# KatiaJDL/CenterPoly

Hardware: AMD Instinct MI355X
Metric: inference img/s @2048x1024 DLA-34 (1 GPU) (higher is better)
Workload: dtype f32 I/O; split-bf16 x3 contraction (a*b ~ ah*bh + ah*bl + al*bh on bf16 MFMA, ~2^-16 per product) in the convolutions, the heads and DCNv2; f32 accumulate; 1 GPU; BASELINE config 2: DLA-34 + DCNv2, 1x3x1024x2048 synthetic, 16-vertex cartesian head, K=128, forward + sigmoid + NMS/top-k/decode; parallelism=single

## Files before the change

### centerpoly_amd/_C.py

```python
import ctypes
import os
from ctypes import POINTER, Structure, c_char_p, c_float, c_int32, c_int64, c_size_t, c_void_p

import torch

_HERE = os.path.dirname(os.path.abspath(__file__))
LIB_PATH = os.path.join(_HERE, "csrc", "libcenterpoly_hip.so")

CP_OK = 0
REP = {"cartesian": 0, "polar": 1, "polar_fixed": 2}
HEATMAP_UMICH, HEATMAP_ELLIPSE = 0, 1
L1_PLAIN, L1_POLAR, L1_POLAR_FIXED, L1_RELU20, L1_SMOOTH = 0, 1, 2, 3, 4
DCN_BWD_EXACT_F32, DCN_BWD_NARROW_TILES = 1, 2
DCN_CONTRACTION = {"f32": 0, "bf16x3": 1, "bf16x3_region": 3}


class DcnShape(Structure):
    _fields_ = [(n, c_int32) for n in ("B", "Cin", "H", "W", "Cout", "kh", "kw", "stride", "pad",
                                       "dil", "deformable_groups")]


class TargetShape(Structure):
    _fields_ = [(n, c_int32) for n in ("B", "max_objs", "nbr_points", "num_classes", "out_h", "out_w",
                                       "rep", "no_reorder_flip")]
# ... 76 lines not shown
    "cp_polydet_targets_ex": (c_int32, [POINTER(TargetShape), c_int32] + [_P] * 19 + [_P, c_size_t, _P]),
    "cp_polydet_dense_targets": (c_int32, [POINTER(TargetShape), _P, _P, c_size_t, _P, _P, _P]),
    "cp_conv_direct_supported": (c_int32, [c_int32] * 5),
    "cp_conv_direct_wgrad_supported": (c_int32, [c_int32] * 5),
    "cp_conv_direct_wgrad": (c_int32, [_P, _P, _P] + [c_int32] * 8 + [_P]),
    "cp_conv_direct_forward": (c_int32, [_P, _P, _P, _P] + [c_int32] * 9 + [_P]),
    "cp_conv_direct_forward_ex": (c_int32, [_P, _P, _P, _P] + [c_int32] * 10 + [_P]),
    "cp_conv3x3_mfma_supported": (c_int32, [c_int32] * 4),
    "cp_conv3x3_mfma_weight_bytes": (c_size_t, [c_int32] * 2),
    "cp_conv3x3_mfma_prepare": (c_int32, [_P, c_int32, c_int32, c_int32, _P, _P]),
    "cp_conv3x3_mfma_forward": (c_int32, [_P, _P, _P, _P, _P] + [c_int32] * 6 + [_P]),
    "cp_conv_mfma_weight_bytes": (c_size_t, [c_int32] * 3),
    "cp_conv_mfma_prepare": (c_int32, [_P, c_int32, c_int32, c_int32, c_int32, _P, _P]),
    "cp_conv3x3_s2_wgrad_supported": (c_int32, [c_int32] * 4),
    "cp_conv3x3_s2_wgrad": (c_int32, [_P, _P, _P] + [c_int32] * 5 + [_P]),
    "cp_conv7x7_c3_supported": (c_int32, [c_int32] * 4),
    "cp_conv7x7_c3_weight_bytes": (c_size_t, [c_int32]),
    "cp_conv7x7_c3_prepare": (c_int32, [_P, c_int32, _P, _P]),
    "cp_conv7x7_c3_forward": (c_int32, [_P, _P, _P, _P] + [c_int32] * 6 + [_P]),
    "cp_conv_mfma_prepare_blocks": (c_int32, [c_int32] * 3),
    "cp_conv_mfma_prepare_batch": (c_int32, [_P, c_int32, c_int32, _P]),
    "cp_conv_mfma_forward": (c_int32, [_P, _P, c_int32, _P, _P, _P, _P] + [c_int32] * 6 + [_P]),
    "cp_conv_mfma_forward_strided": (c_int32, [_P, _P, c_int32, _P, _P, _P, _P] + [c_int32] * 7 + [_P]),
    "cp_dla_base_pair_supported": (c_int32, [c_int32] * 2),
    "cp_dla_base_pair_forward": (c_int32, [_P] * 6 + [c_int32] * 3 + [_P]),
    "cp_conv_mfma_forward_split": (c_int32, [_P, c_int32, _P, _P, _P, _P] + [c_int32] * 9 + [_P]),
    "cp_activation_split": (c_int32, [_P, _P] + [c_int32] * 4 + [_P]),
    "cp_activation_unsplit": (c_int32, [_P, _P] + [c_int32] * 4 + [_P]),
    "cp_conv_mfma_input_grad_relu_workspace_bytes": (c_size_t, [c_int32] * 4),
    "cp_conv_mfma_input_grad_relu": (c_int32, [_P] * 5 + [c_int32] * 6 + [_P, c_size_t, _P]),
    "cp_conv3x3_s2_input_grad": (c_int32, [_P, _P, _P, _P] + [c_int32] * 5 + [_P]),
    "cp_conv3x3_mfma_wgrad_supported": (c_int32, [c_int32] * 4),
    "cp_conv3x3_mfma_wgrad": (c_int32, [_P, _P, _P] + [c_int32] * 5 + [_P]),
    "cp_conv_mfma_wgrad": (c_int32, [_P, _P, _P] + [c_int32] * 6 + [_P]),
    "cp_heads_fused_w2_bytes": (c_size_t, [c_int32]),
    "cp_heads_fused_prepare_w2": (c_int32, [_P, c_int32, c_int32, _P, _P]),
    "cp_heads_fused_forward": (c_int32, [_P, _P, _P, _P, _P, _P, _P] + [c_int32] * 6 + [_P]),
    "cp_maxpool2x2_forward": (c_int32, [_P, _P] + [c_int32] * 4 + [_P]),
    "cp_maxpool2x2_backward": (c_int32, [_P, _P, _P] + [c_int32] * 4 + [_P]),
    "cp_conv1x1_act_forward": (c_int32, [_P, c_int64, _P, c_int32, _P, _P, _P, c_int32, c_int32, c_int32, c_int64, _P]),
    "cp_soft_nms": (c_int32, [_P, c_int32, c_int32, c_float, c_float, c_float, c_int32]),
    "cp_soft_nms_device": (c_int32, [_P, c_int32, _P, _P, c_int32, c_float, c_float, c_float, c_int32, _P, _P]),
    "cp_merge_detections_workspace_bytes": (c_size_t, [c_int32] * 4),
    "cp_merge_detections": (c_int32, [_P] + [c_int32] * 6 + [c_float] * 3 + [c_int32, _P, _P, _P, c_size_t, _P]),
    "cp_polydet_decode_workspace_bytes": (c_size_t, [c_int32] * 5),
    "cp_polydet_decode": (c_int32, [_P, _P, _P, _P] + [c_int32] * 7 + [_P, _P, _P, _P, c_size_t, _P]),
# ... 138 lines not shown
```

### centerpoly_amd/csrc/conv_mfma.hip

```cpp
#include "cp_common.h"

#include <type_traits>

namespace {

typedef __bf16 bf16x8 __attribute__((ext_vector_type(8)));
typedef __bf16 bf16x4 __attribute__((ext_vector_type(4)));
typedef unsigned u32x4 __attribute__((ext_vector_type(4)));
typedef unsigned u32x2 __attribute__((ext_vector_type(2)));

#ifndef CP_CVABL
#define CP_CVABL 0
#endif
#ifdef CP_CVSTAMP
#define CVSTAMP(i) do { if ((i) < 16) stamp[i] = __builtin_amdgcn_s_memtime(); } while (0)
#else
#define CVSTAMP(i) do { } while (0)
#endif
constexpr int KC = 32;
constexpr int TW = 32;
constexpr unsigned OOB = 0xFFFFFFF0u;

__device__ __forceinline__ void wperm_element(const float* __restrict__ w, bf16x8* __restrict__ wp, int M, int K, int nchunk,
                                              int taps, int transposed, int e) {
  const int lane = e & 63;
  int r = e >> 6;
  const int hl = r & 1;
  r >>= 1;
  const int tap = r % taps;
  r /= taps;
  const int chunk = r % nchunk, ct = r / nchunk;
  const int m = ct * 16 + (lane & 15);
  bf16x8 o;
#pragma unroll
  for (int j = 0; j < 8; ++j) {
    const int k = chunk * KC + 8 * (lane >> 4) + j;
    float v = 0.f;
    if (m < M && k < K) {
      if (transposed == 6) {
        v = w[((long long)k * M + m) * 9 + tap];
// ... 33 lines not shown
  v += dpp(v, std::integral_constant<int, 0xB1>{});
  v += dpp(v, std::integral_constant<int, 0x4E>{});
  v += dpp(v, std::integral_constant<int, 0x141>{});
  v += dpp(v, std::integral_constant<int, 0x140>{});
  return v;
}

constexpr int MAXSRC = 4;
struct CvArgs {
  const float* xsrc[MAXSRC];
  int csrc[MAXSRC];
  const bf16x8* wp;
  const float* bias;
  const float* res;
  float* out;
  int Cin, H, W, Ho, Wo, Cout, nchunk, ncot, tiles_x, relu;
  const float* mask;
  float* colsum;
  int Hf, Wf;
  const bf16x8* xpre = nullptr;
  long long pre_plane = 0;
  int out_split = 0;
  long long out_plane = 0;
};

template <int MT, int RW, int TAPS, int KS = 1, int ST = 1, bool IG2 = false, bool PRE = false, bool OSPLIT = false>
__global__ __launch_bounds__(256 * KS, KS > 1 ? (ST > 1 && TAPS == 9 ? 1 : 4) : 2) void conv_mfma_kernel(CvArgs a) {
  static_assert(!IG2 || (TAPS == 9 && KS == 1 && ST == 1), "IG2: 3x3, stride-1 staging, no split-K");
  static_assert(!PRE || (TAPS == 9 && ST == 1 && !IG2), "PRE: 3x3 / stride 1 forward");
  static_assert(!OSPLIT || !IG2, "split planes out: forward forms");
  constexpr bool TRD = !IG2 && !OSPLIT;
  constexpr int NCLS = IG2 ? 4 : 1;
#ifdef CP_CVSTAMP
  unsigned long long stamp[16];
  const unsigned long long rt0 = __builtin_amdgcn_s_memrealtime();
  int sti = 1;
#endif
  CVSTAMP(0);
  constexpr int S = TAPS == 1 ? 1 : ST;
  constexpr int SUB = TAPS == 1 ? ST : 1;
  constexpr int HALO = TAPS == 9 ? 1 : 0, LW = S * TW + (TAPS == 9 ? 3 : 1) - S;
  constexpr int TH = 4 * RW, LH = S * TH + (TAPS == 9 ? 3 : 1) - S, NT = 2 * RW, PLANE = 4 * LH * LW;
  constexpr int UNITS = PLANE, ITERS = (UNITS + 255) / 256, SB = ITERS <= 6 ? ITERS : 5;
  constexpr int RED = (KS - 1) * 256 * MT * NT;
  constexpr int XS_F = KS * 2 * PLANE;
  __shared__ bf16x8 Xall[XS_F > RED ? XS_F : RED];
// ... 30 lines not shown
  f32x4 (&acc)[MT][NT] = accs[0];

  const long long tstride = (long long)a.nchunk * TAPS * 2 * 64;
  const bf16x8* wq = a.wp + (long long)cot * MT * tstride + lane;
  bf16x8 af[MT][2];
  {
    const bf16x8* fq = wq + (long long)(min(grp, a.nchunk - 1) * TAPS * 2) * 64;
#pragma unroll
    for (int m = 0; m < MT; ++m) {
      af[m][0] = fq[m * tstride];
      af[m][1] = fq[m * tstride + 64];
    }
  }

  const int bbase = (g * LH + S * wid * RW) * LW + S * c;

  int src = 0, src_c0 = 0;
  auto load = [&](int chunk, int i0, auto& v) {
    while (src + 1 < MAXSRC && chunk * KC >= src_c0 + a.csrc[src] && a.csrc[src + 1] > 0) {
      src_c0 += a.csrc[src];
      ++src;
    }
    const int cs = a.csrc[src];
    const __amdgpu_buffer_rsrc_t rs_x = __builtin_amdgcn_make_buffer_rsrc(
        const_cast<float*>(a.xsrc[src] + (long long)b * cs * HW), 0, (int)((unsigned)cs * (unsigned)HW * 4u), 0x00020000);
    const unsigned cb = (unsigned)(chunk * KC - src_c0) * cstep;
    constexpr int N = sizeof(v) / sizeof(v[0]);
#pragma unroll
    for (int i = 0; i < N; ++i) {
      const unsigned o = (i0 + i >= ITERS || soff[(i0 + i) % ITERS] == OOB) ? OOB : soff[(i0 + i) % ITERS] + cb;
#pragma unroll
      for (int j = 0; j < 8; ++j)
        v[i][j] = (CP_CVABL & 2) ? (float)(o + j) : __builtin_bit_cast(
            float, __builtin_amdgcn_raw_buffer_load_b32(rs_x, o == OOB ? OOB : o + j * cstep, 0, 0));
    }
  };
  auto store = [&](int i0, auto& v) {
    constexpr int N = sizeof(v) / sizeof(v[0]);
#pragma unroll
    for (int i = 0; i < N; ++i) {
      const int u = tid + (i0 + i) * 256;
      if (i0 + i < ITERS && u < UNITS) {
        bf16x8 h, l;
#pragma unroll
        for (int j = 0; j < 8; ++j) {
          const __bf16 hh = (__bf16)v[i][j];
          h[j] = hh;
          l[j] = (__bf16)(v[i][j] - (float)hh);
        }
        Xs[u] = h;
// ... 18 lines not shown
    }
  };
  auto store_pre = [&](int i0, auto& vh, auto& vl) {
    constexpr int N = sizeof(vh) / sizeof(vh[0]);
#pragma unroll
    for (int i = 0; i < N; ++i) {
      const int u = tid + (i0 + i) * 256;
      if (i0 + i < ITERS && u < UNITS) {
        Xs[u] = __builtin_bit_cast(bf16x8, vh[i]);
        Xs[PLANE + u] = __builtin_bit_cast(bf16x8, vl[i]);
      }
    }
  };
  auto bread = [&](int tap, bf16x8 (&bh)[NT], bf16x8 (&bl)[NT]) {
    const int dy = IG2 ? (tap / 3 == 0 ? 2 : 1) : tap / 3, dx = IG2 ? (tap % 3 == 0 ? 2 : 1) : tap % 3;
#pragma unroll
    for (int n = 0; n < NT; ++n) {
      const int idx = bbase + (S * (n >> 1) + dy) * LW + S * (n & 1) * 16 + dx;
      bh[n] = (CP_CVABL & 4) ? af[n % MT][0] : Xs[idx];
      bl[n] = (CP_CVABL & 4) ? af[n % MT][1] : Xs[PLANE + idx];
    }
  };

  for (int chunk = grp; chunk - grp < a.nchunk; chunk += KS) {
    const bool active = chunk < a.nchunk;
    __syncthreads();
#ifdef CP_CVSTAMP
    CVSTAMP(sti); ++sti;
#endif
    if (active && !(CP_CVABL & 16)) {
#pragma unroll
      for (int i0 = 0; i0 < ITERS; i0 += SB) {
        if constexpr (PRE) {
          u32x4 vh[SB], vl[SB];
          load_pre(chunk, i0, vh, vl);
          store_pre(i0, vh, vl);
        } else {
          float v[SB][8];
          load(chunk, i0, v);
          store(i0, v);
        }
      }
    }
#ifdef CP_CVSTAMP
    CVSTAMP(sti); ++sti;
#endif
    __syncthreads();
#ifdef CP_CVSTAMP
    CVSTAMP(sti); ++sti;
#endif
    if (!active) continue;

#pragma unroll
    for (int tap = 0; tap < TAPS; ++tap) {
      const int cls = IG2 ? (tap / 3 != 1) * 2 + (tap % 3 != 1) : 0;
      bf16x8 an[MT][2];
      {
        const int nfrag = tap < TAPS - 1 ? chunk * TAPS + tap + 1
                                         : (chunk + KS < a.nchunk ? (chunk + KS) * TAPS : chunk * TAPS + tap);
        const bf16x8* nq = wq + (long long)(nfrag * 2) * 64;
#pragma unroll
        for (int m = 0; m < MT; ++m) {
          an[m][0] = (CP_CVABL & 1) ? af[m][0] : nq[m * tstride];
          an[m][1] = (CP_CVABL & 1) ? af[m][1] : nq[m * tstride + 64];
        }
      }
      {
        bf16x8 bh[NT], bl[NT];
        bread(tap, bh, bl);
#pragma unroll
        for (int m = 0; m < MT; ++m)
#pragma unroll
          for (int n = 0; n < NT; ++n) {
            f32x4& d = accs[cls][m][n];
// ... 284 lines not shown
      else if (Cout <= 32 && wgs(2, 16) >= 448) launch(conv_mfma_kernel<2, 4, 9, 1, 1, false, PRE, OS>, 2, 16, 1);
      else if (wgs(2, 8) >= 320) launch(conv_mfma_kernel<2, 2, 9, 1, 1, false, PRE, OS>, 2, 8, 1);
      else if (wgs(2, 4) < 384 && a.nchunk >= 8) launch(conv_mfma_kernel<2, 1, 9, 4, 1, false, PRE, OS>, 2, 4, 4);
      else if (wgs(2, 4) < 768 && a.nchunk >= 4) launch(conv_mfma_kernel<2, 1, 9, 2, 1, false, PRE, OS>, 2, 4, 2);
      else launch(conv_mfma_kernel<2, 1, 9, 1, 1, false, PRE, OS>, 2, 4, 1);
    };
    if (a.xpre && a.out_split) pick(std::true_type{}, std::true_type{});
    else if (a.xpre) pick(std::true_type{}, std::false_type{});
    else if (a.out_split) pick(std::false_type{}, std::true_type{});
    else pick(std::false_type{}, std::false_type{});
  } else {
    if (Cout > 32 && wgs(4, 8) >= 448) launch(conv_mfma_kernel<4, 2, 1>, 4, 8, 1);
    else if (wgs(2, 8) >= 320) launch(conv_mfma_kernel<2, 2, 1>, 2, 8, 1);
    else if (wgs(2, 4) < 384 && a.nchunk >= 8) launch(conv_mfma_kernel<2, 1, 1, 4>, 2, 4, 4);
    else if (wgs(2, 4) < 768 && a.nchunk >= 4) launch(conv_mfma_kernel<2, 1, 1, 2>, 2, 4, 2);
    else launch(conv_mfma_kernel<2, 1, 1>, 2, 4, 1);
  }
  return cp_launch_status();
}

static int conv_forward_impl(const float* const* xs, const int32_t* cs, int32_t nsrc, const void* wperm, const float* bias,
                             const float* residual, const float* mask, float* colsum, float* out, int32_t B, int32_t H,
                             int32_t W, int32_t Cout, int32_t taps, int32_t stride, int32_t relu, void* stream,
                             int* tiles_out = nullptr, int x_split = 0, int out_split = 0) {
  hipStream_t st = (hipStream_t)stream;
  CP_CHECK_ARG(xs && cs && wperm && out && B >= 1 && nsrc >= 1 && nsrc <= MAXSRC && (taps == 1 || taps == 9));
  if (stride != 1 && stride != 2) return CP_EUNSUPPORTED;
  CvArgs a;
  int Cin = 0;
  for (int i = 0; i < MAXSRC; ++i) {
    a.xsrc[i] = i < nsrc ? xs[i] : nullptr;
    a.csrc[i] = i < nsrc ? cs[i] : 0;
    if (i < nsrc) {
      CP_CHECK_ARG(xs[i] && cs[i] >= 1);
      if (nsrc > 1 && cs[i] % KC != 0) return CP_EUNSUPPORTED;
      if (!cp_conv3x3_mfma_supported(cs[i], Cout, H, W)) return CP_EUNSUPPORTED;
      Cin += cs[i];
    }
  }
  a.wp = (const bf16x8*)wperm;
  a.bias = bias;
  a.res = residual;
  a.out = out;
  a.Cin = Cin;
  a.H = H;
  a.W = W;
  a.Cout = Cout;
  a.Ho = (H - 1) / stride + 1;
  a.Wo = (W - 1) / stride + 1;
  a.nchunk = (Cin + KC - 1) / KC;
  a.tiles_x = (a.Wo + TW - 1) / TW;
  a.relu = relu;
  a.Hf = a.Ho; a.Wf = a.Wo;
  a.mask = mask; a.colsum = colsum;
  if ((long long)a.Ho * a.Wo * 64 * 4 >= 0x7FFFFFF0ll) return CP_EUNSUPPORTED;
  if (x_split) {
    if (nsrc != 1 || taps != 9 || stride != 1 || Cin % KC != 0) return CP_EUNSUPPORTED;
    a.xpre = reinterpret_cast<const bf16x8*>(xs[0]);
    a.pre_plane = (long long)B * (Cin / 8) * H * W;
// ... 47 lines not shown
  CP_CHECK_ARG(x && in && B >= 1 && C >= 8 && H >= 1 && W >= 1);
  if (C % 8 != 0) return CP_EUNSUPPORTED;
  const long long HW = (long long)H * W, plane = (long long)B * (C / 8) * HW;
  if (plane >= 0x7FFFFFFFll * 256) return CP_EUNSUPPORTED;
  hipLaunchKernelGGL(activation_unsplit_kernel, dim3((unsigned)((plane + 255) / 256)), dim3(256), 0, (hipStream_t)stream,
                     (const bf16x8*)in, x, HW, plane);
  return cp_launch_status();
}

int cp_conv_mfma_forward_split(const void* x, int32_t x_split, const void* wperm, const float* bias, const float* residual,
                               void* out, int32_t out_split, int32_t B, int32_t Cin, int32_t H, int32_t W, int32_t Cout,
                               int32_t taps, int32_t stride, int32_t relu, void* stream) {
  const float* xs[1] = {reinterpret_cast<const float*>(x)};
  const int32_t cs[1] = {Cin};
  return conv_forward_impl(xs, cs, 1, wperm, bias, residual, nullptr, nullptr, reinterpret_cast<float*>(out), B, H, W, Cout,
                           taps, stride, relu, stream, nullptr, x_split ? 1 : 0, out_split ? 1 : 0);
}

int cp_conv_mfma_forward_strided(const float* const* xs, const int32_t* cs, int32_t nsrc, const void* wperm,
                                 const float* bias, const float* residual, float* out, int32_t B, int32_t H, int32_t W,
                                 int32_t Cout, int32_t taps, int32_t stride, int32_t relu, void* stream) {
  return conv_forward_impl(xs, cs, nsrc, wperm, bias, residual, nullptr, nullptr, out, B, H, W, Cout, taps, stride, relu,
                           stream);
}

size_t cp_conv_mfma_input_grad_relu_workspace_bytes(int32_t B, int32_t Cin, int32_t H, int32_t W) {
  if (B < 1 || Cin < 1 || H < 1 || W < 1) return 0;
  return (size_t)B * ((W + TW - 1) / TW) * ((H + 3) / 4) * 8 * Cin * sizeof(float);
}

int cp_conv_mfma_input_grad_relu(const float* grad_out, const void* wperm_t, const float* y, float* grad_y,
                                 float* grad_bias, int32_t B, int32_t Cin, int32_t H, int32_t W, int32_t Cout,
                                 int32_t taps, void* workspace, size_t workspace_bytes, void* stream) {
  CP_CHECK_ARG(grad_out && y && grad_y && (!grad_bias || workspace));
  if (grad_bias && workspace_bytes < cp_conv_mfma_input_grad_relu_workspace_bytes(B, Cin, H, W)) return CP_EWORKSPACE;
  const float* xs[1] = {grad_out};
  const int32_t cs[1] = {Cout};
  int tiles = 0;
  const int rc = conv_forward_impl(xs, cs, 1, wperm_t, nullptr, nullptr, y, grad_bias ? (float*)workspace : nullptr, grad_y,
                                   B, H, W, Cin, taps, 1, 0, stream, &tiles);
  if (rc != CP_OK || !grad_bias) return rc;
  hipLaunchKernelGGL(colsum_reduce_kernel, dim3((Cin + 63) / 64, 32), dim3(256), 0, (hipStream_t)stream,
                     (const float*)workspace, B * tiles * 8, Cin, grad_bias);
  return cp_launch_status();
}

// ... 290 lines not shown
```

### centerpoly_amd/models/networks/conv3x3.py

```python

import weakref

import torch
import torch.nn.functional as F

from ... import _C
from .prepared import prepared

_ENABLED = True
_WGRAD = True
MIN_CIN = 24
MIN_WORKGROUPS = 128


def _workgroups(B, cout, H, W):
    return B * ((W + 31) // 32) * ((H + 3) // 4) * ((cout + 31) // 32)


def _fills(B, cin, cout, H, W):
    n = _workgroups(B, cout, H, W)
    return n >= MIN_WORKGROUPS or (cin >= 256 and n >= 16)


def usable_shape(x, cout):
    if not (_ENABLED and x.is_cuda and x.dtype == torch.float32 and x.dim() == 4):
        return False
    B, cin, H, W = x.shape
    return cin >= MIN_CIN and bool(_C.lib().cp_conv3x3_mfma_supported(cin, cout, H, W)) \
        and _fills(B, cin, cout, H, W)


def usable(conv, x):
    k = conv.kernel_size
    if not (k in ((3, 3), (1, 1)) and conv.padding == (k[0] // 2, k[0] // 2) and conv.dilation == (1, 1)
# ... 83 lines not shown

def _permute(weight, cin, cout, code):
    L = _C.lib()
    taps = weight.shape[2] * weight.shape[3]
    wp = torch.empty(L.cp_conv_mfma_weight_bytes(cin, cout, taps), dtype=torch.uint8, device=weight.device)
    _C.check(L.cp_conv_mfma_prepare(_C.ptr(weight), cin, cout, taps, code, _C.ptr(wp), _C.stream()), "cp_conv_mfma_prepare")
    return wp


def _launch(x, wp, bias, residual, cout, relu, taps=9, stride=1):
    B, cin, H, W = x.shape
    out = torch.empty((B, cout, (H - 1) // stride + 1, (W - 1) // stride + 1), dtype=torch.float32, device=x.device)
    tag = ("conv3x3_fwd" if stride == 1 else "conv3x3s2_fwd") if taps == 9 else "conv1x1_fwd"
    end = _C.kernel_timer.start((tag, cin, cout, H, W, B)) if _C.kernel_timer is not None else None
    ptrs, chans = (_C.c_void_p * 1)(x.data_ptr()), (_C.c_int32 * 1)(cin)
    _C.check(_C.lib().cp_conv_mfma_forward_strided(ptrs, chans, 1, _C.ptr(wp), _C.ptr(bias), _C.ptr(residual),
                                                   _C.ptr(out), B, H, W, cout, taps, stride, 1 if relu else 0,
                                                   _C.stream()), "cp_conv_mfma_forward_strided")
    if end is not None:
        end.record()
    return out


def conv_infer(xs, owner, w, bias=None, residual=None, relu=False, conv=None, slot="conv", x_split=False,
               out_split=False):
    k = tuple(w.shape[2:])
    if not _ENABLED or k not in ((1, 1), (3, 3)):
        return None
    if (x_split or out_split) and (len(xs) != 1 or k != (3, 3) or (out_split and residual is not None)
                                   or (x_split and xs[0].shape[1] % 32) or (out_split and w.shape[0] % 8)):
        return None
    stride = 1
    if conv is not None:
        if not (conv.stride in ((1, 1), (2, 2)) and conv.padding == (k[0] // 2, k[0] // 2)
                and conv.dilation == (1, 1) and conv.groups == 1 and conv.padding_mode == "zeros"):
            return None
        stride = conv.stride[0]
    x0 = xs[0]
    if not all(x.is_cuda and x.dtype == torch.float32 and x.dim() == 4 and x.shape[0] == x0.shape[0]
               and x.shape[2:] == x0.shape[2:] for x in xs) or len(xs) > 4:
        return None
    cs = [x.shape[1] for x in xs]
    cin, cout = sum(cs), w.shape[0]
    B, _, H, W = x0.shape
    Ho, Wo = (H - 1) // stride + 1, (W - 1) // stride + 1
    L = _C.lib()
    if cin != w.shape[1] or cin < MIN_CIN or (len(xs) > 1 and any(c % 32 for c in cs)) \
            or not all(L.cp_conv3x3_mfma_supported(c, cout, H, W) for c in cs) \
            or not _fills(B, cin, cout, Ho, Wo) or (residual is not None and not residual.is_contiguous()):
        return None
    taps = k[0] * k[1]
    wp, _ = prepared(owner, slot, (w,), lambda: _permute(w.contiguous(), cin, cout, 0))
    xs = [x.contiguous() for x in xs]
    out = torch.empty((B, cout, Ho, Wo), dtype=torch.float32, device=x0.device)
    ptrs = (_C.c_void_p * len(xs))(*[x.data_ptr() for x in xs])
    chans = (_C.c_int32 * len(xs))(*cs)
    tag = "conv3x3_fwd" if taps == 9 and stride == 1 else ("conv3x3s2_fwd" if taps == 9 else "conv1x1_fwd")
    end = _C.kernel_timer.start((tag, cin, cout, H, W, B)) if _C.kernel_timer is not None else None
    if x_split or out_split:
        if x_split and stride != 1:
            return None
        _C.check(L.cp_conv_mfma_forward_split(_C.ptr(xs[0]), 1 if x_split else 0, _C.ptr(wp), _C.ptr(bias),
                                              _C.ptr(residual), _C.ptr(out), 1 if out_split else 0, B, cin, H, W, cout,
                                              taps, stride, 1 if relu else 0, _C.stream()), "cp_conv_mfma_forward_split")
    else:
        _C.check(L.cp_conv_mfma_forward_strided(ptrs, chans, len(xs), _C.ptr(wp), _C.ptr(bias), _C.ptr(residual),
                                                _C.ptr(out), B, H, W, cout, taps, stride, 1 if relu else 0, _C.stream()),
                 "cp_conv_mfma_forward_strided")
    if end is not None:
        end.record()
    return out


def block_infer(x, conv1, wb1, conv2, wb2, skip):
    planes = wb1[0].shape[0]
    if not (_ENABLED and x.is_cuda and planes % 32 == 0 and tuple(wb1[0].shape[2:]) == (3, 3)
            and tuple(wb2[0].shape[2:]) == (3, 3) and conv2.stride == (1, 1)):
        return None
    B, _, H, W = x.shape
    s = conv1.stride[0]
    Ho, Wo = (H - 1) // s + 1, (W - 1) // s + 1
    if planes < MIN_CIN or not _fills(B, planes, planes, Ho, Wo) \
            or not _C.lib().cp_conv3x3_mfma_supported(planes, planes, Ho, Wo) or (skip is not None and not skip.is_contiguous()):
        return None
    y = conv_infer([x], conv1, wb1[0], wb1[1], None, True, conv=conv1, out_split=True)
    if y is None:
        return None
    z = conv_infer([y], conv2, wb2[0], wb2[1], skip, True, conv=conv2, x_split=True)
    if z is None:
        raise _C.NativeError("block_infer: the second convolution refused a split tensor its first convolution wrote")
    return z
# ... 329 lines not shown
```

### centerpoly_amd/models/networks/pose_dla_dcn.py

```python
import math
import os

import numpy as np
import torch
import torch.nn.functional as F
from torch import nn

from ... import _C
from .DCNv2.dcn_v2 import DCN, conv_bias
from . import conv3x3
from .conv3x3 import conv_infer, conv_raw
from .prepared import prepared, release_inference

HEADS_FUSED = True
CONV_DIRECT_WGRAD = True

BN_MOMENTUM = 0.1


def _bn(c):
    return nn.BatchNorm2d(c, momentum=BN_MOMENTUM)



def _fold_conv_bn(conv, bn):
    with torch.no_grad():
        scale = bn.weight * torch.rsqrt(bn.running_var + bn.eps)
        w = (conv.weight * scale.view(-1, 1, 1, 1)).contiguous()
        b = bn.bias - bn.running_mean * scale
        if conv.bias is not None:
            b = b + conv.bias * scale
    return w, b.contiguous()


def _use_folded(m):
    return getattr(m, "_folded", None) is not None and not m.training and not torch.is_grad_enabled()

# ... 136 lines not shown
    return y


class _MaxPool2x2Fn(torch.autograd.Function):

    @staticmethod
    def forward(ctx, x):
        B, C, H, W = x.shape
        out = torch.empty((B, C, H // 2, W // 2), dtype=torch.float32, device=x.device)
        _C.check(_C.lib().cp_maxpool2x2_forward(_C.ptr(x), _C.ptr(out), B, C, H, W, _C.stream()), "cp_maxpool2x2_forward")
        ctx.save_for_backward(x)
        return out

    @staticmethod
    def backward(ctx, go):
        (x,) = ctx.saved_tensors
        B, C, H, W = x.shape
        gx = torch.empty_like(x)
        _C.check(_C.lib().cp_maxpool2x2_backward(_C.ptr(x), _C.ptr(go.contiguous()), _C.ptr(gx), B, C, H, W,
                                                 _C.stream()), "cp_maxpool2x2_backward")
        return gx


def downsample2(pool, x):
    if (x.is_cuda and x.dtype == torch.float32 and x.dim() == 4 and pool.kernel_size in (2, (2, 2))
            and pool.stride in (2, (2, 2)) and pool.padding in (0, (0, 0)) and not pool.ceil_mode
            and x.shape[0] * x.shape[1] <= 65535 and x.shape[2] >= 2 and x.shape[3] >= 2):
        return _MaxPool2x2Fn.apply(x.contiguous())
    return pool(x)


class _BiasRelu(torch.autograd.Function):

    @staticmethod
    def forward(ctx, y_raw, bias):
        B, C, H, W = y_raw.shape
        _C.check(_C.lib().cp_bias_act_inplace(_C.ptr(y_raw), _C.ptr(bias), None, B, C, H * W, 1, _C.stream()),
                 "cp_bias_act_inplace")
        ctx.mark_dirty(y_raw)
        ctx.save_for_backward(y_raw)
        return y_raw

    @staticmethod
    def backward(ctx, go):
        (y,) = ctx.saved_tensors
        go = go.contiguous()
        B, C, H, W = y.shape
        g = torch.empty_like(go)
        gb = _C.zeros((C,), y.device)
        _C.check(_C.lib().cp_bias_relu_backward(_C.ptr(y), _C.ptr(go), _C.ptr(g), _C.ptr(gb), B, C, H * W,
# ... 111 lines not shown
        else:
            y = bn_act(self.bn1, conv_train(self.conv1, x), relu=True)
        return bn_act(self.bn2, conv_train(self.conv2, y), relu=True, residual=skip)


class Root(nn.Module):
    def __init__(self, in_channels, out_channels, kernel_size, residual):
        super().__init__()
        self.conv = nn.Conv2d(in_channels, out_channels, 1, 1, (kernel_size - 1) // 2, bias=False)
        self.bn = _bn(out_channels)
        self.relu = nn.ReLU(inplace=True)
        self.residual = residual

    def fold(self):
        self._folded = _fold_conv_bn(self.conv, self.bn)

    def forward(self, *xs):
        if _use_folded(self):
            res = xs[0] if self.residual else None
            if xs[0].is_cuda:
                y = conv_infer(list(xs), self.conv, self._folded[0], self._folded[1], res, True, conv=self.conv)
                if y is not None:
                    return y
            return _conv_folded(torch.cat(xs, 1), self.conv, self._folded, relu=True, residual=res)
        y = conv3x3.concat_conv1x1(self.conv, xs) if (self.training and xs[0].is_cuda) else None
        if y is None:
            y = conv_train(self.conv, torch.cat(xs, 1))
        return bn_act(self.bn, y, relu=True, residual=xs[0] if self.residual else None)


class Tree(nn.Module):

    def __init__(self, levels, block, in_channels, out_channels, stride=1, level_root=False,
                 root_dim=0, root_kernel_size=1, dilation=1, root_residual=False):
        super().__init__()
        root_dim = root_dim or 2 * out_channels
        if level_root:
            root_dim += in_channels
        self.levels, self.level_root, self.root_dim = levels, level_root, root_dim
        if levels == 1:
            self.tree1 = block(in_channels, out_channels, stride, dilation=dilation)
            self.tree2 = block(out_channels, out_channels, 1, dilation=dilation)
            self.root = Root(root_dim, out_channels, root_kernel_size, root_residual)
        else:
            kw = dict(root_kernel_size=root_kernel_size, dilation=dilation,
                      root_residual=root_residual)
            self.tree1 = Tree(levels - 1, block, in_channels, out_channels, stride, root_dim=0, **kw)
            self.tree2 = Tree(levels - 1, block, out_channels, out_channels,
                              root_dim=root_dim + out_channels, **kw)
        self.downsample = nn.MaxPool2d(stride, stride=stride) if stride > 1 else None
        self.project = None
        if in_channels != out_channels:
            self.project = nn.Sequential(nn.Conv2d(in_channels, out_channels, 1, 1, bias=False),
                                         _bn(out_channels))
        self.project_is_dead = levels > 1 and self.project is not None
        if self.project_is_dead:
            for prm in self.project.parameters():
                prm.requires_grad_(False)

    def fold(self):
        self._folded = _fold_conv_bn(self.project[0], self.project[1]) if self.project is not None \
            else None

    def forward(self, x, residual=None, children=None):
        children = [] if children is None else children
        bottom = x if self.downsample is None else downsample2(self.downsample, x)
        if self.project is None:
            residual = bottom
        elif self.project_is_dead:
            residual = None
            if self.training:
                with torch.no_grad():
                    if bottom.is_cuda:
                        bn_act(self.project[1], conv_train(self.project[0], bottom), relu=False)
                    else:
                        self.project(bottom)
        elif _use_folded(self):
            residual = _conv_folded(bottom, self.project[0], self._folded)
        else:
            residual = bn_act(self.project[1], conv_train(self.project[0], bottom), relu=False)
        if self.level_root:
            children.append(bottom)
        x1 = self.tree1(x, residual)
        if self.levels == 1:
            return self.root(self.tree2(x1), x1, *children)
        children.append(x1)
        return self.tree2(x1, children=children)

# ... 380 lines not shown
```

### include/centerpoly_hip.h

```cpp
#ifndef CENTERPOLY_HIP_H
#define CENTERPOLY_HIP_H

#include <stddef.h>
#include <stdint.h>

#ifdef __cplusplus
extern "C" {
#endif

#define CP_ABI_VERSION 3

enum {
  CP_OK = 0,
  CP_EINVAL = -1,
  CP_EUNSUPPORTED = -2,
  CP_EWORKSPACE = -3,
  CP_EHIP = -4
};

enum { CP_REP_CARTESIAN = 0, CP_REP_POLAR = 1, CP_REP_POLAR_FIXED = 2 };

enum {
  CP_DCN_F32 = 0,
  CP_DCN_BF16X3 = 1,
// ... 78 lines not shown
int cp_conv3x3_mfma_supported(int32_t Cin, int32_t Cout, int32_t H, int32_t W);
size_t cp_conv3x3_mfma_weight_bytes(int32_t Cin, int32_t Cout);
int cp_conv3x3_mfma_prepare(const float* weight, int32_t Cin, int32_t Cout, int32_t transposed, void* wperm,
                            void* stream);
int cp_conv3x3_mfma_forward(const float* x, const void* wperm, const float* bias, const float* residual, float* out,
                            int32_t B, int32_t Cin, int32_t H, int32_t W, int32_t Cout, int32_t relu, void* stream);

size_t cp_conv_mfma_weight_bytes(int32_t Cin, int32_t Cout, int32_t taps);
int cp_conv_mfma_prepare(const float* weight, int32_t Cin, int32_t Cout, int32_t taps, int32_t transposed, void* wperm,
                         void* stream);
typedef struct cp_conv_prepare_job {
  const float* weight;
  void* wperm;
  int32_t Cin, Cout, taps, transposed, first_block, reserved;
} cp_conv_prepare_job;
int32_t cp_conv_mfma_prepare_blocks(int32_t Cin, int32_t Cout, int32_t taps);
int cp_conv_mfma_prepare_batch(const cp_conv_prepare_job* jobs_device, int32_t njobs, int32_t total_blocks, void* stream);
int cp_conv_mfma_forward(const float* const* xs, const int32_t* cs, int32_t nsrc, const void* wperm, const float* bias,
                         const float* residual, float* out, int32_t B, int32_t H, int32_t W, int32_t Cout,
                         int32_t taps, int32_t relu, void* stream);
int cp_conv_mfma_forward_strided(const float* const* xs, const int32_t* cs, int32_t nsrc, const void* wperm,
                                 const float* bias, const float* residual, float* out, int32_t B, int32_t H, int32_t W,
                                 int32_t Cout, int32_t taps, int32_t stride, int32_t relu, void* stream);
int cp_dla_base_pair_supported(int32_t H, int32_t W);
int cp_dla_base_pair_forward(const float* x, const float* w0, const float* b0, const float* w1, const float* b1, float* out,
                             int32_t B, int32_t H, int32_t W, void* stream);
int cp_conv_mfma_forward_split(const void* x, int32_t x_split, const void* wperm, const float* bias, const float* residual,
                               void* out, int32_t out_split, int32_t B, int32_t Cin, int32_t H, int32_t W, int32_t Cout,
                               int32_t taps, int32_t stride, int32_t relu, void* stream);
int cp_activation_split(const float* x, void* out, int32_t B, int32_t C, int32_t H, int32_t W, void* stream);
int cp_activation_unsplit(const void* in, float* x, int32_t B, int32_t C, int32_t H, int32_t W, void* stream);
int cp_conv3x3_s2_wgrad_supported(int32_t Cin, int32_t Cout, int32_t H, int32_t W);
int cp_conv3x3_s2_wgrad(const float* x, const float* grad_out, float* gw, int32_t B, int32_t Cin, int32_t H, int32_t W,
                        int32_t Cout, void* stream);

int cp_conv7x7_c3_supported(int32_t Cout, int32_t H, int32_t W, int32_t stride);
size_t cp_conv7x7_c3_weight_bytes(int32_t Cout);
int cp_conv7x7_c3_prepare(const float* weight, int32_t Cout, void* wperm, void* stream);
int cp_conv7x7_c3_forward(const float* x, const void* wperm, const float* bias, float* out, int32_t B, int32_t H,
                          int32_t W, int32_t Cout, int32_t stride, int32_t relu, void* stream);

size_t cp_conv_mfma_input_grad_relu_workspace_bytes(int32_t B, int32_t Cin, int32_t H, int32_t W);
int cp_conv_mfma_input_grad_relu(const float* grad_out, const void* wperm_t, const float* y, float* grad_y,
                                 float* grad_bias, int32_t B, int32_t Cin, int32_t H, int32_t W, int32_t Cout,
                                 int32_t taps, void* workspace, size_t workspace_bytes, void* stream);
int cp_conv3x3_s2_input_grad(const float* grad_out, const void* wperm_t, const float* residual, float* grad_in, int32_t B,
// ... 203 lines not shown
```

Baseline: 368.4 img/s.

## Fuse 2x2 max-pool into 1x1 conv staging via lazy pooled sources

Adds a PooledSource wrapper so DLA tree downsampling is deferred. A 1x1 projection or root conv whose input is pooled reads the full-resolution tensor and takes the 2x2 max while staging, skipping the separate max-pool kernel and its intermediate tensor when no other consumer needs it. It also adds an optional register-prefetch pipeline for 1x1 convs, which is compiled out by default. The fused load does four scalar, strided buffer reads per element instead of one, which may make staging slower, and other consumers still materialise the pooled tensor.

```diff
diff --git a/centerpoly_amd/_C.py b/centerpoly_amd/_C.py
--- a/centerpoly_amd/_C.py
+++ b/centerpoly_amd/_C.py
@@ -122,6 +122,7 @@
     "cp_conv_mfma_prepare_batch": (c_int32, [_P, c_int32, c_int32, _P]),
     "cp_conv_mfma_forward": (c_int32, [_P, _P, c_int32, _P, _P, _P, _P] + [c_int32] * 6 + [_P]),
     "cp_conv_mfma_forward_strided": (c_int32, [_P, _P, c_int32, _P, _P, _P, _P] + [c_int32] * 7 + [_P]),
+    "cp_conv_mfma_forward_pooled": (c_int32, [_P] * 5 + [c_int32, _P, _P, _P, _P] + [c_int32] * 7 + [_P]),
     "cp_dla_base_pair_supported": (c_int32, [c_int32] * 2),
     "cp_dla_base_pair_forward": (c_int32, [_P] * 6 + [c_int32] * 3 + [_P]),
     "cp_conv_mfma_forward_split": (c_int32, [_P, c_int32, _P, _P, _P, _P] + [c_int32] * 9 + [_P]),
diff --git a/centerpoly_amd/csrc/conv_mfma.hip b/centerpoly_amd/csrc/conv_mfma.hip
--- a/centerpoly_amd/csrc/conv_mfma.hip
+++ b/centerpoly_amd/csrc/conv_mfma.hip
@@ -16,6 +16,9 @@
 #define CVSTAMP(i) do { if ((i) < 16) stamp[i] = __builtin_amdgcn_s_memtime(); } while (0)
 #else
 #define CVSTAMP(i) do { } while (0)
+#endif
+#ifndef CP_CONV1X1_PIPE
+#define CP_CONV1X1_PIPE 0
 #endif
 constexpr int KC = 32;
 constexpr int TW = 32;
@@ -95,6 +98,8 @@
   long long pre_plane = 0;
   int out_split = 0;
   long long out_plane = 0;
+  int pool = 0;
+  int hsrc[MAXSRC] = {0, 0, 0, 0}, wsrc[MAXSRC] = {0, 0, 0, 0};
 };
 
 template <int MT, int RW, int TAPS, int KS = 1, int ST = 1, bool IG2 = false, bool PRE = false, bool OSPLIT = false>
@@ -171,10 +176,37 @@
       ++src;
     }
     const int cs = a.csrc[src];
+    constexpr int N = sizeof(v) / sizeof(v[0]);
+    if (TAPS == 1 && ((a.pool >> src) & 1)) {
+      const unsigned Ws = (unsigned)a.wsrc[src], HWs = (unsigned)a.hsrc[src] * Ws;
+      const __amdgpu_buffer_rsrc_t rs_p = __builtin_amdgcn_make_buffer_rsrc(
+          const_cast<float*>(a.xsrc[src] + (long long)b * cs * HWs), 0, (int)((unsigned)cs * HWs * 4u), 0x00020000);
+      const unsigned cbp = (unsigned)(chunk * KC - src_c0) * HWs * 4u;
+#pragma unroll
+      for (int i = 0; i < N; ++i) {
+        const int u = tid + (i0 + i) * 256;
+        const int col = u % LW, r = (u / LW) % LH, cg = u / (LW * LH);
+        const unsigned gy = (unsigned)(SUB * (y0 + r)), gx = (unsigned)(SUB * (x0 + col));
+        const bool ok = i0 + i < ITERS && soff[(i0 + i) % ITERS] != OOB;
+        const unsigned o = ok ? cbp + ((unsigned)(cg * 8) * HWs + 2u * gy * Ws + 2u * gx) * 4u : OOB;
+#pragma unroll
+        for (int j = 0; j < 8; ++j) {
+          const unsigned oj = o == OOB ? OOB : o + j * HWs * 4u;
+          const unsigned o1 = o == OOB ? OOB : oj + Ws * 4u;
+          auto ld = [&](unsigned off) { return __builtin_bit_cast(float, __builtin_amdgcn_raw_buffer_load_b32(rs_p, off, 0, 0)); };
+          const float p1 = ld(o == OOB ? OOB : oj + 4u), p2 = ld(o1), p3 = ld(o == OOB ? OOB : o1 + 4u);
+          float m = ld(oj);
+          if (p1 > m || p1 != p1) m = p1;
+          if (p2 > m || p2 != p2) m = p2;
+          if (p3 > m || p3 != p3) m = p3;
+          v[i][j] = m;
+        }
+      }
+      return;
+    }
     const __amdgpu_buffer_rsrc_t rs_x = __builtin_amdgcn_make_buffer_rsrc(
         const_cast<float*>(a.xsrc[src] + (long long)b * cs * HW), 0, (int)((unsigned)cs * (unsigned)HW * 4u), 0x00020000);
     const unsigned cb = (unsigned)(chunk * KC - src_c0) * cstep;
-    constexpr int N = sizeof(v) / sizeof(v[0]);
 #pragma unroll
     for (int i = 0; i < N; ++i) {
       const unsigned o = (i0 + i >= ITERS || soff[(i0 + i) % ITERS] == OOB) ? OOB : soff[(i0 + i) % ITERS] + cb;
@@ -239,13 +271,20 @@
     }
   };
 
+  constexpr bool PIPE = TAPS == 1 && CP_CONV1X1_PIPE && !(CP_CVABL & 16);
+  float vp[PIPE ? ITERS : 1][8];
+  if constexpr (PIPE) {
+    if (grp < a.nchunk) load(grp, 0, vp);
+  }
   for (int chunk = grp; chunk - grp < a.nchunk; chunk += KS) {
     const bool active = chunk < a.nchunk;
     __syncthreads();
 #ifdef CP_CVSTAMP
     CVSTAMP(sti); ++sti;
 #endif
-    if (active && !(CP_CVABL & 16)) {
+    if constexpr (PIPE) {
+      if (active) store(0, vp);
+    } else if (active && !(CP_CVABL & 16)) {
 #pragma unroll
       for (int i0 = 0; i0 < ITERS; i0 += SB) {
         if constexpr (PRE) {
@@ -267,6 +306,10 @@
     CVSTAMP(sti); ++sti;
 #endif
     if (!active) continue;
+    if constexpr (PIPE) {
+      if (chunk + KS < a.nchunk) load(chunk + KS, 0, vp);
+      __builtin_amdgcn_sched_barrier(0);
+    }
 
 #pragma unroll
     for (int tap = 0; tap < TAPS; ++tap) {
@@ -597,7 +640,8 @@
 static int conv_forward_impl(const float* const* xs, const int32_t* cs, int32_t nsrc, const void* wperm, const float* bias,
                              const float* residual, const float* mask, float* colsum, float* out, int32_t B, int32_t H,
                              int32_t W, int32_t Cout, int32_t taps, int32_t stride, int32_t relu, void* stream,
-                             int* tiles_out = nullptr, int x_split = 0, int out_split = 0) {
+                             int* tiles_out = nullptr, int x_split = 0, int out_split = 0,
+                             const int32_t* pooled = nullptr, const int32_t* hs = nullptr, const int32_t* ws = nullptr) {
   hipStream_t st = (hipStream_t)stream;
   CP_CHECK_ARG(xs && cs && wperm && out && B >= 1 && nsrc >= 1 && nsrc <= MAXSRC && (taps == 1 || taps == 9));
   if (stride != 1 && stride != 2) return CP_EUNSUPPORTED;
@@ -609,7 +653,17 @@
     if (i < nsrc) {
       CP_CHECK_ARG(xs[i] && cs[i] >= 1);
       if (nsrc > 1 && cs[i] % KC != 0) return CP_EUNSUPPORTED;
-      if (!cp_conv3x3_mfma_supported(cs[i], Cout, H, W)) return CP_EUNSUPPORTED;
+      const bool pl = pooled && pooled[i];
+      if (pooled) {
+        CP_CHECK_ARG(hs && ws && (pl ? hs[i] / 2 == H && ws[i] / 2 == W : hs[i] == H && ws[i] == W));
+        if (pl && taps != 1) return CP_EUNSUPPORTED;
+      }
+      if (!cp_conv3x3_mfma_supported(cs[i], Cout, pl ? hs[i] : H, pl ? ws[i] : W)) return CP_EUNSUPPORTED;
+      if (pl) {
+        a.pool |= 1 << i;
+        a.hsrc[i] = hs[i];
+        a.wsrc[i] = ws[i];
+      }
       Cin += cs[i];
     }
   }
@@ -703,6 +757,15 @@
                                  int32_t Cout, int32_t taps, int32_t stride, int32_t relu, void* stream) {
   return conv_forward_impl(xs, cs, nsrc, wperm, bias, residual, nullptr, nullptr, out, B, H, W, Cout, taps, stride, relu,
                            stream);
+}
+
+int cp_conv_mfma_forward_pooled(const float* const* xs, const int32_t* cs, const int32_t* pooled, const int32_t* hs,
+                                const int32_t* ws, int32_t nsrc, const void* wperm, const float* bias,
+                                const float* residual, float* out, int32_t B, int32_t H, int32_t W, int32_t Cout,
+                                int32_t taps, int32_t stride, int32_t relu, void* stream) {
+  CP_CHECK_ARG(pooled && hs && ws && H >= 1 && W >= 1);
+  return conv_forward_impl(xs, cs, nsrc, wperm, bias, residual, nullptr, nullptr, out, B, H, W, Cout, taps, stride, relu,
+                           stream, nullptr, 0, 0, pooled, hs, ws);
 }
 
 size_t cp_conv_mfma_input_grad_relu_workspace_bytes(int32_t B, int32_t Cin, int32_t H, int32_t W) {
diff --git a/centerpoly_amd/models/networks/conv3x3.py b/centerpoly_amd/models/networks/conv3x3.py
--- a/centerpoly_amd/models/networks/conv3x3.py
+++ b/centerpoly_amd/models/networks/conv3x3.py
@@ -10,6 +10,7 @@
 _ENABLED = True
 _WGRAD = True
 MIN_CIN = 24
+POOL_MAX_COUT = 64
 MIN_WORKGROUPS = 128
 
 
@@ -139,6 +140,22 @@
     return out
 
 
+class PooledSource(object):
+
+    def __init__(self, x, pool):
+        self.x, self._pool, self._t = x, pool, None
+        self.shape = torch.Size((x.shape[0], x.shape[1], x.shape[2] // 2, x.shape[3] // 2))
+
+    def tensor(self):
+        if self._t is None:
+            self._t = self._pool(self.x)
+        return self._t
+
+
+def materialise(x):
+    return x.tensor() if isinstance(x, PooledSource) else x
+
+
 def conv_infer(xs, owner, w, bias=None, residual=None, relu=False, conv=None, slot="conv", x_split=False,
                out_split=False):
     k = tuple(w.shape[2:])
@@ -153,17 +170,25 @@
                 and conv.dilation == (1, 1) and conv.groups == 1 and conv.padding_mode == "zeros"):
             return None
         stride = conv.stride[0]
+    srcs = list(xs)
+    pooled = [isinstance(x, PooledSource) and x._t is None and k == (1, 1) and not (x_split or out_split)
+              and w.shape[0] <= POOL_MAX_COUT
+              and x.x.dim() == 4 and x.x.shape[2] >= 2 and x.x.shape[3] >= 2 for x in xs]
+    xs = [x.x if p else materialise(x) for x, p in zip(xs, pooled)]
+    if not all(x.dim() == 4 for x in xs):
+        return None
+    dims = [(x.shape[2] // 2, x.shape[3] // 2) if p else tuple(x.shape[2:]) for x, p in zip(xs, pooled)]
     x0 = xs[0]
-    if not all(x.is_cuda and x.dtype == torch.float32 and x.dim() == 4 and x.shape[0] == x0.shape[0]
-               and x.shape[2:] == x0.shape[2:] for x in xs) or len(xs) > 4:
+    if not all(x.is_cuda and x.dtype == torch.float32 and x.shape[0] == x0.shape[0] and d == dims[0]
+               for x, d in zip(xs, dims)) or len(xs) > 4:
         return None
     cs = [x.shape[1] for x in xs]
     cin, cout = sum(cs), w.shape[0]
-    B, _, H, W = x0.shape
+    B, (H, W) = x0.shape[0], dims[0]
     Ho, Wo = (H - 1) // stride + 1, (W - 1) // stride + 1
     L = _C.lib()
     if cin != w.shape[1] or cin < MIN_CIN or (len(xs) > 1 and any(c % 32 for c in cs)) \
-            or not all(L.cp_conv3x3_mfma_supported(c, cout, H, W) for c in cs) \
+            or not all(L.cp_conv3x3_mfma_supported(c, cout, x.shape[2], x.shape[3]) for c, x in zip(cs, xs)) \
             or not _fills(B, cin, cout, Ho, Wo) or (residual is not None and not residual.is_contiguous()):
         return None
     taps = k[0] * k[1]
@@ -181,9 +206,23 @@
                                               _C.ptr(residual), _C.ptr(out), 1 if out_split else 0, B, cin, H, W, cout,
                                               taps, stride, 1 if relu else 0, _C.stream()), "cp_conv_mfma_forward_split")
     else:
-        _C.check(L.cp_conv_mfma_forward_strided(ptrs, chans, len(xs), _C.ptr(wp), _C.ptr(bias), _C.ptr(residual),
-                                                _C.ptr(out), B, H, W, cout, taps, stride, 1 if relu else 0, _C.stream()),
-                 "cp_conv_mfma_forward_strided")
+        rc = -2
+        if any(pooled):
+            n = len(xs)
+            rc = L.cp_conv_mfma_forward_pooled(ptrs, chans, (_C.c_int32 * n)(*[int(p) for p in pooled]),
+                                               (_C.c_int32 * n)(*[x.shape[2] for x in xs]),
+                                               (_C.c_int32 * n)(*[x.shape[3] for x in xs]), n, _C.ptr(wp), _C.ptr(bias),
+                                               _C.ptr(residual), _C.ptr(out), B, H, W, cout, taps, stride,
+                                               1 if relu else 0, _C.stream())
+            if rc != -2:
+                _C.check(rc, "cp_conv_mfma_forward_pooled")
+            else:
+                xs = [materialise(s).contiguous() if p else x for s, x, p in zip(srcs, xs, pooled)]
+                ptrs = (_C.c_void_p * n)(*[x.data_ptr() for x in xs])
+        if rc == -2:
+            _C.check(L.cp_conv_mfma_forward_strided(ptrs, chans, len(xs), _C.ptr(wp), _C.ptr(bias), _C.ptr(residual),
+                                                    _C.ptr(out), B, H, W, cout, taps, stride, 1 if relu else 0,
+                                                    _C.stream()), "cp_conv_mfma_forward_strided")
     if end is not None:
         end.record()
     return out
diff --git a/centerpoly_amd/models/networks/pose_dla_dcn.py b/centerpoly_amd/models/networks/pose_dla_dcn.py
--- a/centerpoly_amd/models/networks/pose_dla_dcn.py
+++ b/centerpoly_amd/models/networks/pose_dla_dcn.py
@@ -13,6 +13,7 @@
 from .prepared import prepared, release_inference
 
 HEADS_FUSED = True
+POOL_IN_STAGING = True
 CONV_DIRECT_WGRAD = True
 
 BN_MOMENTUM = 0.1
@@ -195,10 +196,14 @@
         return gx
 
 
+def _pool2x2_native(pool, x):
+    return (x.is_cuda and x.dtype == torch.float32 and x.dim() == 4 and pool.kernel_size in (2, (2, 2))
+            and pool.stride in (2, (2, 2)) and pool.padding in (0, (0, 0)) and not pool.ceil_mode
+            and x.shape[0] * x.shape[1] <= 65535 and x.shape[2] >= 2 and x.shape[3] >= 2)
+
+
 def downsample2(pool, x):
-    if (x.is_cuda and x.dtype == torch.float32 and x.dim() == 4 and pool.kernel_size in (2, (2, 2))
-            and pool.stride in (2, (2, 2)) and pool.padding in (0, (0, 0)) and not pool.ceil_mode
-            and x.shape[0] * x.shape[1] <= 65535 and x.shape[2] >= 2 and x.shape[3] >= 2):
+    if _pool2x2_native(pool, x):
         return _MaxPool2x2Fn.apply(x.contiguous())
     return pool(x)
 
@@ -356,6 +361,7 @@
                 y = conv_infer(list(xs), self.conv, self._folded[0], self._folded[1], res, True, conv=self.conv)
                 if y is not None:
                     return y
+            xs = [conv3x3.materialise(x) for x in xs]
             return _conv_folded(torch.cat(xs, 1), self.conv, self._folded, relu=True, residual=res)
         y = conv3x3.concat_conv1x1(self.conv, xs) if (self.training and xs[0].is_cuda) else None
         if y is None:
@@ -396,8 +402,26 @@
         self._folded = _fold_conv_bn(self.project[0], self.project[1]) if self.project is not None \
             else None
 
-    def forward(self, x, residual=None, children=None):
+    def forward(self, x, residual=None, children=None, pooled=None):
         children = [] if children is None else children
+        if (POOL_IN_STAGING and self.downsample is not None and _use_folded(self) and conv3x3.mfma_enabled()
+                and _pool2x2_native(self.downsample, x)):
+            bottom = pooled if (pooled is not None and pooled.x is x) else \
+                conv3x3.PooledSource(x, lambda t: downsample2(self.downsample, t))
+            residual = None
+            if not self.project_is_dead:
+                residual = conv_infer([bottom], self.project[0], self._folded[0], self._folded[1], None, False,
+                                      conv=self.project[0])
+                if residual is None:
+                    residual = _conv_folded(bottom.tensor(), self.project[0], self._folded)
+            if self.level_root:
+                children.append(bottom)
+            if self.levels == 1:
+                x1 = self.tree1(x, residual)
+                return self.root(self.tree2(x1), x1, *children)
+            x1 = self.tree1(x, residual, pooled=bottom)
+            children.append(x1)
+            return self.tree2(x1, children=children)
         bottom = x if self.downsample is None else downsample2(self.downsample, x)
         if self.project is None:
             residual = bottom
diff --git a/include/centerpoly_hip.h b/include/centerpoly_hip.h
--- a/include/centerpoly_hip.h
+++ b/include/centerpoly_hip.h
@@ -124,6 +124,10 @@
 int cp_conv_mfma_forward_strided(const float* const* xs, const int32_t* cs, int32_t nsrc, const void* wperm,
                                  const float* bias, const float* residual, float* out, int32_t B, int32_t H, int32_t W,
                                  int32_t Cout, int32_t taps, int32_t stride, int32_t relu, void* stream);
+int cp_conv_mfma_forward_pooled(const float* const* xs, const int32_t* cs, const int32_t* pooled, const int32_t* hs,
+                                const int32_t* ws, int32_t nsrc, const void* wperm, const float* bias,
+                                const float* residual, float* out, int32_t B, int32_t H, int32_t W, int32_t Cout,
+                                int32_t taps, int32_t stride, int32_t relu, void* stream);
 int cp_dla_base_pair_supported(int32_t H, int32_t W);
 int cp_dla_base_pair_forward(const float* x, const float* w0, const float* b0, const float* w1, const float* b1, float* out,
                              int32_t B, int32_t H, int32_t W, void* stream);
```

Result: no change. 369.3 img/s (median of 6 runs) (+0.2%).
